# Auxeno/diamond-ppo

Hardware: AMD Instinct MI355X
Metric: env-steps/sec (GAE+update) on synthetic [128 x num_envs] buffers (higher is better)
Workload: dtype f32; 1 GPU; LunarLander-v3 PPO: learn() = old-policy eval + GAE + adv-norm + 4x8 minibatch Adam steps; rollout_steps=128, num_envs_per_gpu=8192, num_envs_total=8192, obs_dim=8, act_dim=4, continuous=False, hidden=64, batch_per_learn=1048576, minibatch=131072, parallelism=env-axis dp1, exchange=none, minibatches=reference

## Files before the change

### diamond-ppo_amd/csrc/mlp.hip

```cpp
#include "actdraw.h"
#include "common.h"

namespace dppo {
namespace {

constexpr int H = 64;
constexpr int SW = H + 4;
constexpr int kThreads = 512;
constexpr int kWaves = kThreads / kWave;
constexpr float kLogSqrt2Pi = 0.91893853320467274178f;
constexpr float kTS = 2.8853900817779268f;
constexpr int kQueueCap = 256;
constexpr int kMatchRound = 4;

struct LdsLayout {
  static constexpr int W2 = 0, Wa = H * SW, Wc = 2 * H * SW;
  static constexpr int Wo = 3 * H * SW;
  static constexpr int kWoCap = 16 * H;
  static constexpr int Wv = Wo + kWoCap;
  static constexpr int b1 = Wv + H, b2 = b1 + H, ba = b2 + H, bc = ba + H;
  static constexpr int bo = bc + H, ls = bo + 32;
  static constexpr int bv = ls + 32;
  static constexpr int W1 = bv + 4;
  static constexpr int kS1Max = 36;
  static constexpr int weights_end = W1 + H * kS1Max;
  static constexpr int queue = weights_end;
  static constexpr int total = queue + kWaves * kQueueCap + 2 * kWaves;
  int S1;
};
static_assert(LdsLayout::W1 % 4 == 0 && LdsLayout::Wo % 4 == 0, "16-B aligned images");

struct KArgs {
  LdsLayout L;
  ParamOffsets po;
  const float* params;
  const float* obs;
  const void* actions;
  const float* next_obs;
  float *logp, *values, *next_values;
  int64_t n;
  int D, D8, nq1, A, R;
  int q4;
  int64_t row;
};

__host__ __device__ inline int align4(int x) { return (x + 3) & ~3; }

LdsLayout make_layout(const MlpShape& sh) {
  LdsLayout L{};
  L.S1 = sh.D8 + 4;
  return L;
}

__device__ __forceinline__ float* opaque_base(float* p) {
  int z;
  asm volatile("s_mov_b32 %0, 0" : "=s"(z));
  return p + z;
}

__device__ __forceinline__ f32x16 mfma(float a, float b, f32x16 c) {
  return __builtin_amdgcn_mfma_f32_32x32x2f32(a, b, c, 0, 0, 0);
}

__device__ __forceinline__ void load_weights(float* lds, const KArgs& a, int tid) {
  const float* P = a.params;
  const LdsLayout& L = a.L;
  for (int k = tid; k < H * L.S1; k += kThreads) {
    const int o = k / L.S1, c = k % L.S1;
    lds[L.W1 + k] = c < a.D ? P[a.po.W1 + o * a.D + c] * kTS : 0.0f;
  }
  for (int k = tid; k < H * H; k += kThreads) {
    const int o = k >> 6, c = k & 63;
    lds[L.W2 + o * SW + c] = P[a.po.W2 + k] * kTS;
    lds[L.Wa + o * SW + c] = P[a.po.Wa + k] * kTS;
    lds[L.Wc + o * SW + c] = P[a.po.Wc + k] * kTS;
  }
  for (int k = tid; k < a.A * H; k += kThreads) lds[L.Wo + k] = P[a.po.Wo + k];
  for (int k = tid; k < H; k += kThreads) {
    lds[L.Wv + k] = P[a.po.Wv + k];
    lds[L.b1 + k] = P[a.po.b1 + k] * kTS;
    lds[L.b2 + k] = P[a.po.b2 + k] * kTS;
    lds[L.ba + k] = P[a.po.ba + k] * kTS;
    lds[L.bc + k] = P[a.po.bc + k] * kTS;
  }
  for (int k = tid; k < 32; k += kThreads) {
    lds[L.bo + k] = k < a.A ? P[a.po.bo + k] : 0.0f;
    lds[L.ls + k] = (a.po.ls >= 0 && k < a.A) ? P[a.po.ls + k] : 0.0f;
  }
  if (tid < 4) lds[L.bv + tid] = tid == 0 ? P[a.po.bv] : 0.0f;
}

__device__ __forceinline__ f32x16 bias_block(const float* b, int ob, int h) {
  f32x16 acc;
  const float* bp = b + ob * 32 + 4 * h;
#pragma unroll
  for (int q = 0; q < 4; ++q) {
    const f32x4 v = *(const f32x4*)(bp + 8 * q);
    acc[4 * q + 0] = v[0];
    acc[4 * q + 1] = v[1];
    acc[4 * q + 2] = v[2];
    acc[4 * q + 3] = v[3];
  }
  return acc;
}

__device__ __forceinline__ void tanh_inplace(f32x16& x) {
  f32x2 e[8];
#pragma unroll
  for (int r = 0; r < 16; ++r) e[r >> 1][r & 1] = __builtin_amdgcn_exp2f(x[r]);
#pragma unroll
  for (int p = 0; p < 8; ++p) e[p] = e[p] + 1.0f;
#pragma unroll
  for (int r = 0; r < 16; ++r) e[r >> 1][r & 1] = __builtin_amdgcn_rcpf(e[r >> 1][r & 1]);
#pragma unroll
  for (int p = 0; p < 8; ++p) {
    const f32x2 y = __builtin_elementwise_fma((f32x2)(-2.0f), e[p], (f32x2)(1.0f));
    x[2 * p] = y[0];
    x[2 * p + 1] = y[1];
  }
}

__device__ __forceinline__ float half_sum(float part) {
  const auto p = __builtin_amdgcn_permlane32_swap(__float_as_uint(part), __float_as_uint(part),
                                                  false, false);
  return __uint_as_float(p[0]) + __uint_as_float(p[1]);
}

__device__ __forceinline__ void dense_tanh(f32x16 (&out)[2], const float* W, const float* b,
                                           const f32x16 (&x)[2], int l31, int h) {
#pragma unroll
  for (int ob = 0; ob < 2; ++ob) {
    f32x16 acc = bias_block(b, ob, h);
    const float* wp = W + (ob * 32 + l31) * SW + 4 * h;
#pragma unroll
    for (int kb = 0; kb < 2; ++kb) {
#pragma unroll
      for (int q = 0; q < 4; ++q) {
        const f32x4 w = *(const f32x4*)(wp + kb * 32 + 8 * q);
        acc = mfma(w[0], x[kb][4 * q + 0], acc);
        acc = mfma(w[1], x[kb][4 * q + 1], acc);
        acc = mfma(w[2], x[kb][4 * q + 2], acc);
        acc = mfma(w[3], x[kb][4 * q + 3], acc);
      }
    }
    tanh_inplace(acc);
    out[ob] = acc;
    __builtin_amdgcn_sched_barrier(0);
  }
}

__device__ __forceinline__ void dense1_tanh(f32x16 (&out)[2], const float* W1, int S1,
                                            const float* b, const f32x16& x0, int nq1, int l31,
                                            int h) {
#pragma unroll
  for (int ob = 0; ob < 2; ++ob) {
    f32x16 acc = bias_block(b, ob, h);
    const float* wp = W1 + (ob * 32 + l31) * S1 + 4 * h;
#pragma unroll
    for (int q = 0; q < 4; ++q) {
      if (q < nq1) {
        const f32x4 w = *(const f32x4*)(wp + 8 * q);
        acc = mfma(w[0], x0[4 * q + 0], acc);
        acc = mfma(w[1], x0[4 * q + 1], acc);
        acc = mfma(w[2], x0[4 * q + 2], acc);
        acc = mfma(w[3], x0[4 * q + 3], acc);
      }
    }
    tanh_inplace(acc);
    out[ob] = acc;
  }
}







template <int AMAX>
__device__ __forceinline__ void heads(float (&out)[AMAX], const float* Wo, const float* bo,
                                      int A, const f32x16 (&x)[2], int h) {
#pragma unroll
  for (int a = 0; a < AMAX; ++a) {
    float part = 0.0f;
    if (a < A) {
      const float* wp = Wo + a * H + 4 * h;
      f32x2 pa = (f32x2)(0.0f), pb = (f32x2)(0.0f);
#pragma unroll
      for (int fb = 0; fb < 2; ++fb) {
        f32x4 w[4];
#pragma unroll
        for (int q = 0; q < 4; ++q)
          if (AMAX <= 8) w[q] = *(const f32x4*)(wp + fb * 32 + 8 * q);
#pragma unroll
        for (int q = 0; q < 4; ++q) {
          const f32x4 wq = AMAX <= 8 ? w[q] : *(const f32x4*)(wp + fb * 32 + 8 * q);
          pa = __builtin_elementwise_fma((f32x2){wq[0], wq[1]},
                                         (f32x2){x[fb][4 * q + 0], x[fb][4 * q + 1]}, pa);
          pb = __builtin_elementwise_fma((f32x2){wq[2], wq[3]},
                                         (f32x2){x[fb][4 * q + 2], x[fb][4 * q + 3]}, pb);
        }
      }
      const f32x2 pp = pa + pb;
      part = pp[0] + pp[1];
    }
    out[a] = half_sum(part) + bo[a];
  }
}

__device__ __forceinline__ float value_head(const float* Wv, float bv, const f32x16 (&x)[2],
                                            int h) {
  const float* wp = Wv + 4 * h;
  f32x2 pa = (f32x2)(0.0f), pb = (f32x2)(0.0f);
#pragma unroll
  for (int fb = 0; fb < 2; ++fb) {
    f32x4 w[4];
#pragma unroll
    for (int q = 0; q < 4; ++q) w[q] = *(const f32x4*)(wp + fb * 32 + 8 * q);
#pragma unroll
    for (int q = 0; q < 4; ++q) {
      pa = __builtin_elementwise_fma((f32x2){w[q][0], w[q][1]},
                                     (f32x2){x[fb][4 * q + 0], x[fb][4 * q + 1]}, pa);
      pb = __builtin_elementwise_fma((f32x2){w[q][2], w[q][3]},
                                     (f32x2){x[fb][4 * q + 2], x[fb][4 * q + 3]}, pb);
    }
  }
  const f32x2 pp = pa + pb;
  return half_sum(pp[0] + pp[1]) + bv;
}



__device__ __forceinline__ f32x16 load_x0_obs(const float* o, int D, int nq1, bool valid, int h,
                                              bool q4) {
  f32x16 x;
  if (q4) {
#pragma unroll
    for (int q = 0; q < 4; ++q) {
      if (q < nq1) {
        const int f = 8 * q + 4 * h;
        const f32x4 v = *(const f32x4*)(o + (f < D ? f : D - 4));
        const bool on = valid && f < D;
#pragma unroll
        for (int j = 0; j < 4; ++j) x[4 * q + j] = on ? v[j] : 0.0f;
      }
    }
  } else {
#pragma unroll
    for (int q = 0; q < 4; ++q) {
      if (q < nq1) {
#pragma unroll
        for (int j = 0; j < 4; ++j) {
          const int f = 8 * q + 4 * h + j;
          x[4 * q + j] = (valid && f < D) ? o[f] : 0.0f;
        }
      }
    }
  }
  return x;
}

template <int AMAX, bool CONT>
__global__ __launch_bounds__(kThreads, 4) void eval_kernel(KArgs a) {
  extern __shared__ __attribute__((aligned(16))) float lds_[];
  const int tid = threadIdx.x, lane = tid & 63, wave = tid >> 6;
  const int l31 = lane & 31, h = lane >> 5;
  load_weights(lds_, a, tid);
  __syncthreads();
  const LdsLayout& L = a.L;
  const float bv = lds_[L.bv];
  const int64_t ntiles = (a.n + 31) / 32;
  const int qbase = L.queue + __builtin_amdgcn_readfirstlane(wave) * kQueueCap;
  int qh = 0, qn = 0;
  auto critic_tile = [&](bool qv, int64_t k) {
    float* lds = opaque_base(lds_);
    f32x16 x[2], y[2];
    x[0] = load_x0_obs(a.next_obs + k * a.D, a.D, a.nq1, qv, h, a.q4);
    dense1_tanh(y, lds + L.W1, L.S1, lds + L.b1, x[0], a.nq1, l31, h);
    dense_tanh(x, lds + L.W2, lds + L.b2, y, l31, h);
    dense_tanh(y, lds + L.Wc, lds + L.bc, x, l31, h);
    const float nv = value_head(lds + L.Wv, bv, y, h);
    if (qv && h == 0) a.next_values[k] = nv;
  };
  auto critic_queue = [&](int cnt) {
    const bool qv = l31 < cnt;
    const int64_t k = qv ? ((const int32_t*)lds_)[qbase + ((qh + l31) & (kQueueCap - 1))] : 0;
    critic_tile(qv, k);
    qh = (qh + cnt) & (kQueueCap - 1);
    qn -= cnt;
  };
  for (int64_t tile = (int64_t)blockIdx.x * kWaves + wave; tile < ntiles;
       tile += (int64_t)gridDim.x * kWaves) {
    float* lds = opaque_base(lds_);
    const int64_t i = tile * 32 + l31;
    const bool valid = i < a.n;
    const int64_t ic = valid ? i : 0;
    const int act_d = CONT ? 0 : ((const int32_t*)a.actions)[ic];
    f32x16 x[2], y[2];
    x[0] = load_x0_obs(a.obs + ic * a.D, a.D, a.nq1, valid, h, a.q4);
    dense1_tanh(y, lds + L.W1, L.S1, lds + L.b1, x[0], a.nq1, l31, h);
    dense_tanh(x, lds + L.W2, lds + L.b2, y, l31, h);
    dense_tanh(y, lds + L.Wc, lds + L.bc, x, l31, h);
    const float v = value_head(lds + L.Wv, bv, y, h);
    dense_tanh(y, lds + L.Wa, lds + L.ba, x, l31, h);
    float out[AMAX];
    heads<AMAX>(out, lds + L.Wo, lds + L.bo, a.A, y, h);
    float logp;
    if (CONT) {
      const float* act = (const float*)a.actions + ic * a.A;
      logp = 0.0f;
#pragma unroll
      for (int k = 0; k < AMAX; ++k) {
        if (k < a.A) {
          const float ls = lds[L.ls + k];
          const float sc = expf(ls);
          const float d = act[k] - out[k];
          logp += -(d * d) / (2.0f * (sc * sc)) - logf(sc) - kLogSqrt2Pi;
        }
      }
    } else {
      const int act = act_d;
      float mx = out[0];
#pragma unroll
      for (int k = 1; k < AMAX; ++k)
        if (k < a.A) mx = fmaxf(mx, out[k]);
      float se = 0.0f, za = out[0];
#pragma unroll
      for (int k = 0; k < AMAX; ++k)
        if (k < a.A) {
          se += expf(out[k] - mx);
          if (k == act) za = out[k];
        }
      logp = za - (mx + logf(se));
    }
    if (a.row > 0) {
      const int64_t ip = i - a.row;
      bool need_p = false, need_s = false;
      if (valid && h == 0) {
        need_s = i + a.row >= a.n;
        if (ip >= 0) {
          bool m = true;
          const uint32_t* p = (const uint32_t*)(a.next_obs + ip * a.D);
          const uint32_t* o = (const uint32_t*)(a.obs + ic * a.D);
          if (a.q4) {
            for (int f0 = 0; f0 < a.D; f0 += 4 * kMatchRound) {
              u32x4 pv[kMatchRound], ov[kMatchRound];
#pragma unroll
              for (int j = 0; j < kMatchRound; ++j) {
                const int f = f0 + 4 * j < a.D ? f0 + 4 * j : a.D - 4;
                pv[j] = *(const u32x4*)(p + f);
                ov[j] = *(const u32x4*)(o + f);
              }
#pragma unroll
              for (int j = 0; j < kMatchRound; ++j)
                m = m & (pv[j][0] == ov[j][0]) & (pv[j][1] == ov[j][1]) & (pv[j][2] == ov[j][2]) &
                    (pv[j][3] == ov[j][3]);
            }
          } else {
            for (int f0 = 0; f0 < a.D; f0 += kMatchRound) {
              uint32_t pv[kMatchRound], ov[kMatchRound];
#pragma unroll
              for (int j = 0; j < kMatchRound; ++j) {
                const int f = f0 + j < a.D ? f0 + j : a.D - 1;
                pv[j] = p[f];
                ov[j] = o[f];
              }
#pragma unroll
              for (int j = 0; j < kMatchRound; ++j) m = m & (pv[j] == ov[j]);
            }
          }
          if (m) a.next_values[ip] = v;
          need_p = !m;
        }
        a.logp[i] = logp;
        a.values[i] = v;
      }
      const uint64_t bp = __ballot(need_p), bs = __ballot(need_s);
      const uint64_t below = (1ull << lane) - 1ull;
      int32_t* qr = (int32_t*)lds_ + qbase;
      if (need_p) qr[(qh + qn + __popcll(bp & below)) & (kQueueCap - 1)] = (int32_t)ip;
      const int np = __builtin_amdgcn_readfirstlane(__popcll(bp));
      if (need_s) qr[(qh + qn + np + __popcll(bs & below)) & (kQueueCap - 1)] = (int32_t)i;
      qn = __builtin_amdgcn_readfirstlane(qn + np + __popcll(bs));
      while (qn >= 32) critic_queue(32);
      continue;
    }
    x[0] = load_x0_obs(a.next_obs + ic * a.D, a.D, a.nq1, valid, h, a.q4);
    dense1_tanh(y, lds + L.W1, L.S1, lds + L.b1, x[0], a.nq1, l31, h);
    dense_tanh(x, lds + L.W2, lds + L.b2, y, l31, h);
    dense_tanh(y, lds + L.Wc, lds + L.bc, x, l31, h);
    const float nv = value_head(lds + L.Wv, bv, y, h);
    if (valid && h == 0) {
      a.logp[i] = logp;
      a.values[i] = v;
      a.next_values[i] = nv;
    }
  }
  if (a.row > 0) {
    int* rem = (int*)lds_ + L.queue + kWaves * kQueueCap;
    if (lane == 0) {
      rem[wave] = qn;
      rem[kWaves + wave] = qh;
    }
    __syncthreads();
    int tot = 0;
#pragma unroll
    for (int w = 0; w < kWaves; ++w) tot += rem[w];
    if (32 * wave < tot) {
      const int pos = 32 * wave + l31;
      bool qv = pos < tot;
      int64_t k = 0;
      if (qv) {
        int base = 0;
#pragma unroll
        for (int w = 0; w < kWaves; ++w) {
          const int c = rem[w];
          if (pos >= base && pos < base + c)
            k = ((const int32_t*)lds_)[L.queue + w * kQueueCap +
                                       ((rem[kWaves + w] + pos - base) & (kQueueCap - 1))];
          base += c;
        }
      }
      critic_tile(qv, k);
    }
  }
}

struct ActArgs {
  LdsLayout L;
  ParamOffsets po;
  const float* params;
  const float* obs;
  void* actions;
  float* heads;
  float* env_act;
  int squash;
  float sq_lo[16], sq_half[16], sq_hi[16];
  int64_t n;
  uint32_t seed_lo, seed_hi, ctr_lo, ctr_hi;
  int D, D8, nq1, A;
  int q4;
};

__device__ __forceinline__ void load_weights_actor(float* lds, const ActArgs& a, int tid) {
  const float* P = a.params;
  const LdsLayout& L = a.L;
  for (int k = tid; k < H * L.S1; k += kThreads) {
    const int o = k / L.S1, c = k % L.S1;
    lds[L.W1 + k] = c < a.D ? P[a.po.W1 + o * a.D + c] * kTS : 0.0f;
  }
  for (int k = tid; k < H * H; k += kThreads) {
    const int o = k >> 6, c = k & 63;
    lds[L.W2 + o * SW + c] = P[a.po.W2 + k] * kTS;
    lds[L.Wa + o * SW + c] = P[a.po.Wa + k] * kTS;
  }
  for (int k = tid; k < a.A * H; k += kThreads) lds[L.Wo + k] = P[a.po.Wo + k];
  for (int k = tid; k < H; k += kThreads) {
    lds[L.b1 + k] = P[a.po.b1 + k] * kTS;
    lds[L.b2 + k] = P[a.po.b2 + k] * kTS;
    lds[L.ba + k] = P[a.po.ba + k] * kTS;
  }
  for (int k = tid; k < 32; k += kThreads) {
    lds[L.bo + k] = k < a.A ? P[a.po.bo + k] : 0.0f;
    lds[L.ls + k] = (a.po.ls >= 0 && k < a.A) ? P[a.po.ls + k] : 0.0f;
  }
}

template <int AMAX, bool CONT>
__global__ __launch_bounds__(kThreads, 4) void act_kernel(ActArgs a) {
  extern __shared__ __attribute__((aligned(16))) float lds_[];
  const int tid = threadIdx.x, lane = tid & 63, wave = tid >> 6;
  const int l31 = lane & 31, h = lane >> 5;
  load_weights_actor(lds_, a, tid);
  __syncthreads();
  const LdsLayout& L = a.L;
  const int64_t ntiles = (a.n + 31) / 32;
  for (int64_t tile = (int64_t)blockIdx.x * kWaves + wave; tile < ntiles;
       tile += (int64_t)gridDim.x * kWaves) {
    float* lds = opaque_base(lds_);
    const int64_t i = tile * 32 + l31;
    const bool valid = i < a.n;
    const int64_t ic = valid ? i : 0;
    f32x16 x[2], y[2];
    x[0] = load_x0_obs(a.obs + ic * a.D, a.D, a.nq1, valid, h, a.q4);
    dense1_tanh(y, lds + L.W1, L.S1, lds + L.b1, x[0], a.nq1, l31, h);
    dense_tanh(x, lds + L.W2, lds + L.b2, y, l31, h);
    dense_tanh(y, lds + L.Wa, lds + L.ba, x, l31, h);
    float out[AMAX];
    heads<AMAX>(out, lds + L.Wo, lds + L.bo, a.A, y, h);
    if (!valid || h != 0) continue;
    if (a.heads) {
#pragma unroll
      for (int k = 0; k < AMAX; ++k)
        if (k < a.A) a.heads[i * a.A + k] = out[k];
    }
    if (!a.actions) continue;
    if (CONT) {
      draw_gaussian<AMAX>(a, out, lds + L.ls, i, (float*)a.actions + i * a.A);
    } else {
      ((int32_t*)a.actions)[i] = draw_categorical<AMAX>(a, out, i);
    }
  }
}

KArgs base_args(const MlpShape& sh, const ParamOffsets& po, const float* params) {
  KArgs k{};
  k.L = make_layout(sh);
  k.po = po;
  k.params = params;
  k.D = sh.D;
  k.D8 = sh.D8;
  k.nq1 = sh.D8 / 8;
  k.A = sh.A;
  k.R = sh.R;
  return k;
}

#define DPPO_DISPATCH(KERNEL, SH, GRID, LDSB, STREAM, ARGS)                                    \
  do {                                                                                       \
    const int A_ = (SH).A;                                                                   \
    const bool C_ = (SH).continuous != 0;                                                    \
    if (A_ <= 2) {                                                                           \
      if (C_) DPPO_LAUNCH((KERNEL<2, true>), GRID, dim3(kThreads), LDSB, STREAM, ARGS); \
      else DPPO_LAUNCH((KERNEL<2, false>), GRID, dim3(kThreads), LDSB, STREAM, ARGS);   \
    } else if (A_ <= 4) {                                                                    \
      if (C_) DPPO_LAUNCH((KERNEL<4, true>), GRID, dim3(kThreads), LDSB, STREAM, ARGS); \
      else DPPO_LAUNCH((KERNEL<4, false>), GRID, dim3(kThreads), LDSB, STREAM, ARGS);   \
    } else if (A_ <= 8) {                                                                    \
      if (C_) DPPO_LAUNCH((KERNEL<8, true>), GRID, dim3(kThreads), LDSB, STREAM, ARGS); \
      else DPPO_LAUNCH((KERNEL<8, false>), GRID, dim3(kThreads), LDSB, STREAM, ARGS);   \
    } else {                                                                                 \
      if (C_) DPPO_LAUNCH((KERNEL<16, true>), GRID, dim3(kThreads), LDSB, STREAM, ARGS); \
      else DPPO_LAUNCH((KERNEL<16, false>), GRID, dim3(kThreads), LDSB, STREAM, ARGS);  \
    }                                                                                        \
  } while (0)

void raise_lds_limits() {
  static const bool done = [] {
#define DPPO_SET(A, C) raise_dyn_lds((const void*)eval_kernel<A, C>);
    DPPO_SET(2, false) DPPO_SET(2, true) DPPO_SET(4, false) DPPO_SET(4, true)
    DPPO_SET(8, false) DPPO_SET(8, true) DPPO_SET(16, false) DPPO_SET(16, true)
#undef DPPO_SET
#define DPPO_SET(A, C) raise_dyn_lds((const void*)act_kernel<A, C>);
    DPPO_SET(2, false) DPPO_SET(2, true) DPPO_SET(4, false) DPPO_SET(4, true)
    DPPO_SET(8, false) DPPO_SET(8, true) DPPO_SET(16, false) DPPO_SET(16, true)
#undef DPPO_SET
    return true;
  }();
  (void)done;
}

int cu_count() {
  static int cus = 0;
  if (cus == 0) {
    int dev = 0;
    if (hipGetDevice(&dev) != hipSuccess ||
        hipDeviceGetAttribute(&cus, hipDeviceAttributeMultiprocessorCount, dev) != hipSuccess ||
        cus <= 0)
      cus = 256;
  }
  return cus;
}

}

int launch_eval(const MlpShape& sh, const ParamOffsets& po, const float* params, const float* obs,
                const void* actions, const float* next_obs, float* logp, float* values,
                float* next_values, int64_t n, hipStream_t s, EvalReuse* reuse) {
  if (n <= 0) return DPPO_OK;
  KArgs k = base_args(sh, po, params);
  if (reuse && reuse->row > 0 && reuse->row < n) k.row = reuse->row;
  k.obs = obs;
  k.actions = actions;
  k.next_obs = next_obs;
  k.q4 = (sh.D % 4 == 0) && ((uintptr_t)obs % 16 == 0) && (!next_obs || (uintptr_t)next_obs % 16 == 0);
  k.logp = logp;
  k.values = values;
  k.next_values = next_values;
  k.n = n;
  const size_t lds = (size_t)k.L.total * sizeof(float);
  raise_lds_limits();
  static int cus = 0;
  if (cus == 0) {
    int dev = 0;
    if (hipGetDevice(&dev) != hipSuccess ||
        hipDeviceGetAttribute(&cus, hipDeviceAttributeMultiprocessorCount, dev) != hipSuccess ||
        cus <= 0)
      cus = 256;
  }
  const int64_t ntiles = (n + 31) / 32;
  int64_t g = (ntiles + kWaves - 1) / kWaves;
  if (g > 2 * cus) g = 2 * cus;
  DPPO_DISPATCH(eval_kernel, sh, dim3((unsigned)g), lds, s, k);
  DPPO_LAUNCH_CHECK();
  return DPPO_OK;
}

int launch_act(const MlpShape& sh, const ParamOffsets& po, const float* params, const float* obs,
               void* actions, int64_t n, uint64_t seed, uint64_t counter, hipStream_t s,
               float* heads, const ActSquash* squash) {
  if (n <= 0) return DPPO_OK;
  ActArgs k{};
  if (squash && squash->env_actions) {
    if (!sh.continuous || sh.A > 16) {
      set_error("tanh squash needs a continuous action space of at most 16 dims");
      return DPPO_EINVAL;
    }
    k.env_act = squash->env_actions;
    k.squash = squash->low && squash->high ? 2 : 1;
    for (int j = 0; j < sh.A && k.squash == 2; ++j) {
      k.sq_lo[j] = squash->low[j];
      k.sq_half[j] = 0.5f * (squash->high[j] - squash->low[j]);
      k.sq_hi[j] = squash->high[j];
    }
  }
  k.L = make_layout(sh);
  k.po = po;
  k.params = params;
  k.obs = obs;
  k.actions = actions;
  k.heads = heads;
  k.n = n;
  k.seed_lo = (uint32_t)seed;
  k.seed_hi = (uint32_t)(seed >> 32);
  k.ctr_lo = (uint32_t)counter;
  k.ctr_hi = (uint32_t)(counter >> 32);
  k.D = sh.D;
  k.D8 = sh.D8;
  k.nq1 = sh.D8 / 8;
  k.A = sh.A;
  k.q4 = (sh.D % 4 == 0) && ((uintptr_t)obs % 16 == 0);
  const size_t lds = (size_t)k.L.total * sizeof(float);
  raise_lds_limits();
  const int64_t ntiles = (n + 31) / 32;
  int64_t g = (ntiles + kWaves - 1) / kWaves;
  if (g > 2 * cu_count()) g = 2 * cu_count();
  DPPO_DISPATCH(act_kernel, sh, dim3((unsigned)g), lds, s, k);
  DPPO_LAUNCH_CHECK();
  return DPPO_OK;
}

}
```

Before: 277.2 million env-steps/s.

## Emulate f32 hidden-layer GEMMs in eval kernel with split-bf16 MFMA

Hidden-layer weights are staged in LDS as three bf16 pieces (hi/mid/lo), and activations are split the same way at runtime. The 64x64 hidden layers then run as six bf16 32x32x16 MFMA products instead of the f32 32x32x2 MFMA chain, approximating f32 accuracy at higher throughput. The larger LDS layout lowers occupancy to one workgroup per CU, which changes launch bounds and grid size. Precision drops slightly because the smallest cross terms are omitted, and the extra split arithmetic and register pressure add cost.

```diff
diff --git a/diamond-ppo_amd/csrc/mlp.hip b/diamond-ppo_amd/csrc/mlp.hip
--- a/diamond-ppo_amd/csrc/mlp.hip
+++ b/diamond-ppo_amd/csrc/mlp.hip
@@ -1,5 +1,7 @@
 #include "actdraw.h"
 #include "common.h"
+
+#include <type_traits>
 
 namespace dppo {
 namespace {
@@ -12,10 +14,20 @@
 constexpr float kTS = 2.8853900817779268f;
 constexpr int kQueueCap = 256;
 constexpr int kMatchRound = 4;
-
-struct LdsLayout {
-  static constexpr int W2 = 0, Wa = H * SW, Wc = 2 * H * SW;
-  static constexpr int Wo = 3 * H * SW;
+#ifdef DPPO_EVAL_F32
+constexpr bool kSplit = false;
+#else
+constexpr bool kSplit = true;
+#endif
+constexpr int PS = H / 2 + 4;
+constexpr int kPiece = H * PS;
+constexpr int kEvalWgPerCu = kSplit ? 1 : 2, kEvalOcc = kSplit ? 2 : 4;
+
+template <bool SPLIT>
+struct LdsLayoutT {
+  static constexpr int kHid = SPLIT ? 3 * kPiece : H * SW;
+  static constexpr int W2 = 0, Wa = kHid, Wc = 2 * kHid;
+  static constexpr int Wo = 3 * kHid;
   static constexpr int kWoCap = 16 * H;
   static constexpr int Wv = Wo + kWoCap;
   static constexpr int b1 = Wv + H, b2 = b1 + H, ba = b2 + H, bc = ba + H;
@@ -28,10 +40,15 @@
   static constexpr int total = queue + kWaves * kQueueCap + 2 * kWaves;
   int S1;
 };
+using LdsLayout = LdsLayoutT<false>;
+using EvalLayout = LdsLayoutT<kSplit>;
 static_assert(LdsLayout::W1 % 4 == 0 && LdsLayout::Wo % 4 == 0, "16-B aligned images");
+static_assert(EvalLayout::W1 % 4 == 0 && EvalLayout::Wo % 4 == 0 && kPiece % 4 == 0 && PS % 4 == 0,
+              "16-B aligned images");
+static_assert(EvalLayout::total * sizeof(float) * kEvalWgPerCu <= 160 * 1024, "LDS per CU");
 
 struct KArgs {
-  LdsLayout L;
+  EvalLayout L;
   ParamOffsets po;
   const float* params;
   const float* obs;
@@ -46,8 +63,9 @@
 
 __host__ __device__ inline int align4(int x) { return (x + 3) & ~3; }
 
-LdsLayout make_layout(const MlpShape& sh) {
-  LdsLayout L{};
+template <class Layout = LdsLayout>
+Layout make_layout(const MlpShape& sh) {
+  Layout L{};
   L.S1 = sh.D8 + 4;
   return L;
 }
@@ -62,18 +80,56 @@
   return __builtin_amdgcn_mfma_f32_32x32x2f32(a, b, c, 0, 0, 0);
 }
 
+typedef __bf16 bf16x2 __attribute__((ext_vector_type(2)));
+typedef __bf16 bf16x8 __attribute__((ext_vector_type(8)));
+
+__device__ __forceinline__ uint32_t pk_bf16(float a, float b) {
+  return __builtin_bit_cast(uint32_t, __builtin_convertvector((f32x2){a, b}, bf16x2));
+}
+
+__device__ __forceinline__ void split_pair(float a, float b, uint32_t& hi, uint32_t& mid,
+                                           uint32_t& lo) {
+  hi = pk_bf16(a, b);
+  a -= __uint_as_float(hi << 16);
+  b -= __uint_as_float(hi & 0xffff0000u);
+  mid = pk_bf16(a, b);
+  a -= __uint_as_float(mid << 16);
+  b -= __uint_as_float(mid & 0xffff0000u);
+  lo = pk_bf16(a, b);
+}
+
+__device__ __forceinline__ void stage_pieces(float* img, const float* W, int tid) {
+  uint16_t* im = (uint16_t*)img;
+  for (int k = tid; k < H * H; k += kThreads) {
+    const int o = k >> 6, c = k & 63;
+    const int f = (c & 32) + 16 * ((c >> 4) & 1) + 8 * ((c >> 2) & 1) + 4 * ((c >> 3) & 1) + (c & 3);
+    uint32_t hi, mid, lo;
+    split_pair(__fmul_rn(W[o * H + f], kTS), 0.0f, hi, mid, lo);
+    const int at = o * (2 * PS) + c;
+    im[at] = (uint16_t)hi;
+    im[2 * kPiece + at] = (uint16_t)mid;
+    im[4 * kPiece + at] = (uint16_t)lo;
+  }
+}
+
 __device__ __forceinline__ void load_weights(float* lds, const KArgs& a, int tid) {
   const float* P = a.params;
-  const LdsLayout& L = a.L;
+  const EvalLayout& L = a.L;
   for (int k = tid; k < H * L.S1; k += kThreads) {
     const int o = k / L.S1, c = k % L.S1;
     lds[L.W1 + k] = c < a.D ? P[a.po.W1 + o * a.D + c] * kTS : 0.0f;
   }
-  for (int k = tid; k < H * H; k += kThreads) {
-    const int o = k >> 6, c = k & 63;
-    lds[L.W2 + o * SW + c] = P[a.po.W2 + k] * kTS;
-    lds[L.Wa + o * SW + c] = P[a.po.Wa + k] * kTS;
-    lds[L.Wc + o * SW + c] = P[a.po.Wc + k] * kTS;
+  if constexpr (kSplit) {
+    stage_pieces(lds + L.W2, P + a.po.W2, tid);
+    stage_pieces(lds + L.Wa, P + a.po.Wa, tid);
+    stage_pieces(lds + L.Wc, P + a.po.Wc, tid);
+  } else {
+    for (int k = tid; k < H * H; k += kThreads) {
+      const int o = k >> 6, c = k & 63;
+      lds[L.W2 + o * SW + c] = P[a.po.W2 + k] * kTS;
+      lds[L.Wa + o * SW + c] = P[a.po.Wa + k] * kTS;
+      lds[L.Wc + o * SW + c] = P[a.po.Wc + k] * kTS;
+    }
   }
   for (int k = tid; k < a.A * H; k += kThreads) lds[L.Wo + k] = P[a.po.Wo + k];
   for (int k = tid; k < H; k += kThreads) {
@@ -147,6 +203,83 @@
     out[ob] = acc;
     __builtin_amdgcn_sched_barrier(0);
   }
+}
+
+struct Pieces {
+  u32x4 hi[4], mid[4], lo[4];
+};
+
+__device__ __forceinline__ void split_act(Pieces& p, const f32x16 (&x)[2]) {
+#pragma unroll
+  for (int s = 0; s < 4; ++s) {
+#pragma unroll
+    for (int j = 0; j < 4; ++j) {
+      uint32_t hi, mid, lo;
+      split_pair(x[s >> 1][8 * (s & 1) + 2 * j], x[s >> 1][8 * (s & 1) + 2 * j + 1], hi, mid, lo);
+      p.hi[s][j] = hi;
+      p.mid[s][j] = mid;
+      p.lo[s][j] = lo;
+    }
+  }
+}
+
+__device__ __forceinline__ f32x16 mfma_bf(u32x4 a, u32x4 b, f32x16 c) {
+  return __builtin_amdgcn_mfma_f32_32x32x16_bf16(__builtin_bit_cast(bf16x8, a),
+                                                 __builtin_bit_cast(bf16x8, b), c, 0, 0, 0);
+}
+
+__device__ __forceinline__ void dense_tanh_split(f32x16 (&out)[2], const float* W, const float* b,
+                                                 const Pieces& x, int l31, int h) {
+#pragma unroll
+  for (int ob = 0; ob < 2; ++ob) {
+    f32x16 B = bias_block(b, ob, h), S;
+#pragma unroll
+    for (int r = 0; r < 16; ++r) S[r] = 0.0f;
+    const float* wp = W + (ob * 32 + l31) * PS + 4 * h;
+    u32x4 wh[4], wm[4], wl[4];
+#pragma unroll
+    for (int s = 0; s < 4; ++s) {
+      wh[s] = *(const u32x4*)(wp + 8 * s);
+      wl[s] = *(const u32x4*)(wp + 2 * kPiece + 8 * s);
+    }
+#pragma unroll
+    for (int s = 0; s < 4; ++s) wm[s] = *(const u32x4*)(wp + kPiece + 8 * s);
+#pragma unroll
+    for (int s = 0; s < 4; ++s) B = mfma_bf(wh[s], x.hi[s], B);
+#pragma unroll
+    for (int s = 0; s < 4; ++s) S = mfma_bf(wl[s], x.hi[s], S);
+#pragma unroll
+    for (int s = 0; s < 4; ++s) S = mfma_bf(wh[s], x.lo[s], S);
+#pragma unroll
+    for (int s = 0; s < 4; ++s) S = mfma_bf(wm[s], x.mid[s], S);
+#pragma unroll
+    for (int s = 0; s < 4; ++s) S = mfma_bf(wm[s], x.hi[s], S);
+#pragma unroll
+    for (int s = 0; s < 4; ++s) S = mfma_bf(wh[s], x.mid[s], S);
+    B = B + S;
+    tanh_inplace(B);
+    out[ob] = B;
+    __builtin_amdgcn_sched_barrier(0);
+  }
+}
+
+struct Blocks {
+  f32x16 v[2];
+};
+using HidIn = std::conditional<kSplit, Pieces, Blocks>::type;
+
+__device__ __forceinline__ void to_input(Pieces& p, const f32x16 (&x)[2]) { split_act(p, x); }
+__device__ __forceinline__ void to_input(Blocks& p, const f32x16 (&x)[2]) {
+  p.v[0] = x[0];
+  p.v[1] = x[1];
+}
+__device__ __forceinline__ void hidden_tanh(f32x16 (&out)[2], const float* W, const float* b,
+                                            const Pieces& x, int l31, int h) {
+  dense_tanh_split(out, W, b, x, l31, h);
+}
+__device__ __forceinline__ void hidden_tanh(f32x16 (&out)[2], const float* W, const float* b,
+                                            const Blocks& x, int l31, int h) {
+  dense_tanh(out, W, b, x.v, l31, h);
 }
 
 __device__ __forceinline__ void dense1_tanh(f32x16 (&out)[2], const float* W1, int S1,
@@ -261,13 +394,13 @@
 }
 
 template <int AMAX, bool CONT>
-__global__ __launch_bounds__(kThreads, 4) void eval_kernel(KArgs a) {
+__global__ __launch_bounds__(kThreads, kEvalOcc) void eval_kernel(KArgs a) {
   extern __shared__ __attribute__((aligned(16))) float lds_[];
   const int tid = threadIdx.x, lane = tid & 63, wave = tid >> 6;
   const int l31 = lane & 31, h = lane >> 5;
   load_weights(lds_, a, tid);
   __syncthreads();
-  const LdsLayout& L = a.L;
+  const EvalLayout& L = a.L;
   const float bv = lds_[L.bv];
   const int64_t ntiles = (a.n + 31) / 32;
   const int qbase = L.queue + __builtin_amdgcn_readfirstlane(wave) * kQueueCap;
@@ -275,10 +408,13 @@
   auto critic_tile = [&](bool qv, int64_t k) {
     float* lds = opaque_base(lds_);
     f32x16 x[2], y[2];
+    HidIn p;
     x[0] = load_x0_obs(a.next_obs + k * a.D, a.D, a.nq1, qv, h, a.q4);
     dense1_tanh(y, lds + L.W1, L.S1, lds + L.b1, x[0], a.nq1, l31, h);
-    dense_tanh(x, lds + L.W2, lds + L.b2, y, l31, h);
-    dense_tanh(y, lds + L.Wc, lds + L.bc, x, l31, h);
+    to_input(p, y);
+    hidden_tanh(x, lds + L.W2, lds + L.b2, p, l31, h);
+    to_input(p, x);
+    hidden_tanh(y, lds + L.Wc, lds + L.bc, p, l31, h);
     const float nv = value_head(lds + L.Wv, bv, y, h);
     if (qv && h == 0) a.next_values[k] = nv;
   };
@@ -297,12 +433,15 @@
     const int64_t ic = valid ? i : 0;
     const int act_d = CONT ? 0 : ((const int32_t*)a.actions)[ic];
     f32x16 x[2], y[2];
+    HidIn p;
     x[0] = load_x0_obs(a.obs + ic * a.D, a.D, a.nq1, valid, h, a.q4);
     dense1_tanh(y, lds + L.W1, L.S1, lds + L.b1, x[0], a.nq1, l31, h);
-    dense_tanh(x, lds + L.W2, lds + L.b2, y, l31, h);
-    dense_tanh(y, lds + L.Wc, lds + L.bc, x, l31, h);
+    to_input(p, y);
+    hidden_tanh(x, lds + L.W2, lds + L.b2, p, l31, h);
+    to_input(p, x);
+    hidden_tanh(y, lds + L.Wc, lds + L.bc, p, l31, h);
     const float v = value_head(lds + L.Wv, bv, y, h);
-    dense_tanh(y, lds + L.Wa, lds + L.ba, x, l31, h);
+    hidden_tanh(y, lds + L.Wa, lds + L.ba, p, l31, h);
     float out[AMAX];
     heads<AMAX>(out, lds + L.Wo, lds + L.bo, a.A, y, h);
     float logp;
@@ -387,8 +526,10 @@
     }
     x[0] = load_x0_obs(a.next_obs + ic * a.D, a.D, a.nq1, valid, h, a.q4);
     dense1_tanh(y, lds + L.W1, L.S1, lds + L.b1, x[0], a.nq1, l31, h);
-    dense_tanh(x, lds + L.W2, lds + L.b2, y, l31, h);
-    dense_tanh(y, lds + L.Wc, lds + L.bc, x, l31, h);
+    to_input(p, y);
+    hidden_tanh(x, lds + L.W2, lds + L.b2, p, l31, h);
+    to_input(p, x);
+    hidden_tanh(y, lds + L.Wc, lds + L.bc, p, l31, h);
     const float nv = value_head(lds + L.Wv, bv, y, h);
     if (valid && h == 0) {
       a.logp[i] = logp;
@@ -505,7 +646,7 @@
 
 KArgs base_args(const MlpShape& sh, const ParamOffsets& po, const float* params) {
   KArgs k{};
-  k.L = make_layout(sh);
+  k.L = make_layout<EvalLayout>(sh);
   k.po = po;
   k.params = params;
   k.D = sh.D;
@@ -590,7 +731,7 @@
   }
   const int64_t ntiles = (n + 31) / 32;
   int64_t g = (ntiles + kWaves - 1) / kWaves;
-  if (g > 2 * cus) g = 2 * cus;
+  if (g > kEvalWgPerCu * cus) g = kEvalWgPerCu * cus;
   DPPO_DISPATCH(eval_kernel, sh, dim3((unsigned)g), lds, s, k);
   DPPO_LAUNCH_CHECK();
   return DPPO_OK;
```

Measured after the change: 273.4 million env-steps/s. -1.3%, worse.
